# SamShue/EKF_SLAM

Measured on AMD Instinct MI355X. Metric: EKF update-steps/sec at N landmarks; HBM GB/s on (I−KH)P vs roofline, higher is better.
Workload: dtype f64

## Files before the change

ekf_slam_amd/csrc/downdate.h:

```cpp
#pragma once

template <typename TS, int T, int kSlab>
__global__ __launch_bounds__(kBlock) void k_downdate(const TS *__restrict__ tiles, TS *__restrict__ dst,
                                                     const int2 *__restrict__ work, int64_t nwork,
                                                     const double *__restrict__ Kp, const double *__restrict__ Gp,
                                                     int64_t pair_stride, int pstart, int pcap, int npairs, TileMap tm) {
    using V2 = typename Vec2<TS>::type;
    constexpr int kPairsPerRow = T / 2;
    constexpr int kRowsPerPass = kBlock / kPairsPerRow;
    constexpr int kSlabsPerTile = T / kSlab;
    constexpr int kPasses = (kSlab + kRowsPerPass - 1) / kRowsPerPass;
    constexpr bool kExact = kRowsPerPass * kPasses == kSlab;
    static_assert(kPasses <= 8, "slab too tall for the register tile");
    const int tid = threadIdx.x;
    const int cp = tid % kPairsPerRow;
    const int r0 = tid / kPairsPerRow;
    const int64_t nitems = nwork * kSlabsPerTile;
    for (int64_t it0 = blockIdx.x; it0 < nitems; it0 += gridDim.x) {
        const int64_t it = tm.reverse ? nitems - 1 - it0 : it0;
        const int64_t w = it / kSlabsPerTile;
        const int slab = (int)(it - w * kSlabsPerTile);
        const int2 ij = work[w];
        const int64_t toff = tm.tile_offset(ij.x, ij.y) + (int64_t)slab * kSlab * T;
        const TS *__restrict__ tp = tiles + toff;
// ... 28 lines not shown
        for (int p = 0; p < kPasses; ++p) {
            const int r = r0 + p * kRowsPerPass;
            if (kExact || r < kSlab) {
                V2 o;
                o.x = (TS)v[p].x; o.y = (TS)v[p].y;
                *reinterpret_cast<V2 *>(td + r * T + 2 * cp) = o;
            }
        }
    }
}

template <typename TS> struct Lane16;
template <> struct Lane16<double> { using type = double2; static constexpr int kCols = 2; };
template <> struct Lane16<float>  { using type = float4;  static constexpr int kCols = 4; };
__device__ __forceinline__ void lane16_unpack(const double2 &t, double *v) { v[0] = t.x; v[1] = t.y; }
__device__ __forceinline__ void lane16_unpack(const float4 &t, double *v) { v[0] = t.x; v[1] = t.y; v[2] = t.z; v[3] = t.w; }
__device__ __forceinline__ void lane16_pack(const double *v, double2 &t) { t.x = v[0]; t.y = v[1]; }
__device__ __forceinline__ void lane16_pack(const double *v, float4 &t) {
    t.x = (float)v[0]; t.y = (float)v[1]; t.z = (float)v[2]; t.w = (float)v[3];
}
__device__ __forceinline__ double lane16_get(const double2 &t, int q) { return q == 0 ? t.x : t.y; }
__device__ __forceinline__ double lane16_get(const float4 &t, int q) { return (double)(q == 0 ? t.x : q == 1 ? t.y : q == 2 ? t.z : t.w); }

__device__ __attribute__((noinline)) void extract_next_row(double *__restrict__ send, int jm, int Ij, int tI, int tJ, int r, int c0, int ncols,
                                                           int T, int world, int rank, double v0, double v1, double v2, double v3) {
    const uint32_t wd = (uint32_t)world;
    const int k0 = (int)(((uint32_t)rank + wd - (uint32_t)Ij % wd) % wd);
    const bool rowtile = tI == Ij, coltile = tJ == Ij, diag = rowtile && coltile;
    for (int q = 0; q < ncols; ++q) {
        const int cc = c0 + q;
        const double val = q == 0 ? v0 : q == 1 ? v1 : q == 2 ? v2 : v3;
        if (rowtile && (r == jm || r == jm + 1)) {
            const int a = r - jm;
            if (!diag || cc <= jm) {
                const int64_t e = (int64_t)((tJ - k0) / world) * T + cc;
                send[2 * e + a] = val;
            }
            if (diag && a == 1 && (cc == jm || cc == jm + 1)) {
                const int64_t e = (int64_t)((Ij - k0) / world) * T + jm + 1;
                send[2 * e + (cc - jm)] = val;
            }
        }
        if (coltile && (cc == jm || cc == jm + 1) && (tI > Ij || r > jm + 1)) {
            const int64_t e = (int64_t)((tI - k0) / world) * T + r;
            send[2 * e + (cc - jm)] = val;
        }
    }
}

struct NoNextRow {};
template <bool kNext> struct NextRowParam { using type = NoNextRow; };
template <> struct NextRowParam<true> { using type = NextRow; };

template <typename TS, int T, int kSlab, bool kXcd, bool kNext = false>
__global__ __launch_bounds__(kBlock) void k_downdate_w(const TS *__restrict__ tiles, TS *__restrict__ dst,
                                                       const int2 *__restrict__ work, int64_t nwork,
                                                       const double *__restrict__ Kp, const double *__restrict__ Gp,
                                                       int64_t pair_stride, int pstart, int pcap, int npairs, TileMap tm,
                                                       typename NextRowParam<kNext>::type nx) {
    using VL = typename Lane16<TS>::type;
    constexpr int kCols = Lane16<TS>::kCols;
    constexpr int kLanesPerRow = T / kCols;
    constexpr int kRowsPerInstr = 64 / kLanesPerRow;
    constexpr int kRowsPerWave = kSlab / 4;
    constexpr int kPasses = kRowsPerWave / kRowsPerInstr;
    constexpr int kSlabsPerTile = T / kSlab;
    static_assert(kLanesPerRow == 64 || kLanesPerRow == 32, "tile edge / storage type combination not supported");
    static_assert(kPasses >= 1 && kPasses <= 8 && kPasses * kRowsPerInstr * 4 == kSlab, "bad slab");
    const int lane = threadIdx.x & 63;
    const int wave = __builtin_amdgcn_readfirstlane(threadIdx.x >> 6);
    const int sub = lane / kLanesPerRow;
    const int cl = lane % kLanesPerRow;
    const int64_t nitems = (kXcd ? 8 : 1) * nwork * kSlabsPerTile;
    const int64_t nv = nwork * kSlabsPerTile;
    for (int64_t it = blockIdx.x; it < nitems; it += gridDim.x) {
        const int64_t vf = kXcd ? (it >> 3) : it;
        const int64_t vi = tm.reverse ? nv - 1 - vf : vf;
        const int64_t w = vi / kSlabsPerTile;
        const int slab = (int)(vi - w * kSlabsPerTile);
        const int2 ij = work[kXcd ? (it & 7) * nwork + w : w];
        if (kXcd && ij.x < 0) continue;
        const int row0 = slab * kSlab + wave * kRowsPerWave;
        const int64_t toff = tm.tile_offset(ij.x, ij.y) + (int64_t)(row0 + sub) * T + kCols * cl;
        const TS *__restrict__ tp = tiles + toff;
        TS *__restrict__ td = dst + toff;
        double v[kPasses][kCols];
#pragma unroll
        for (int p = 0; p < kPasses; ++p) {
            const VL t = *reinterpret_cast<const VL *>(tp + (int64_t)p * kRowsPerInstr * T);
            lane16_unpack(t, v[p]);
        }
        const int64_t gcol = (int64_t)ij.y * T + kCols * cl;
        const int64_t krow = (int64_t)ij.x * T + row0;
        for (int i = 0; i < npairs; ++i) {
            const int64_t so = (int64_t)ring_slot(pstart, i, pcap) * pair_stride;
            const double2 *__restrict__ g2 = reinterpret_cast<const double2 *>(Gp + so) + gcol;
            const double2 *__restrict__ k2 = reinterpret_cast<const double2 *>(Kp + so) + krow;
            double2 g[kCols];
#pragma unroll
            for (int q = 0; q < kCols; ++q) g[q] = g2[q];
#pragma unroll
            for (int p = 0; p < kPasses; ++p) {
                double2 k = k2[p * kRowsPerInstr];
                if (kRowsPerInstr == 2) { const double2 k1 = k2[p * 2 + 1]; if (sub) k = k1; }
#pragma unroll
                for (int q = 0; q < kCols; ++q) v[p][q] = rank2_apply(v[p][q], k, g[q]);
            }
        }
        VL stored[kPasses];
#pragma unroll
        for (int p = 0; p < kPasses; ++p) {
            lane16_pack(v[p], stored[p]);
            *reinterpret_cast<VL *>(td + (int64_t)p * kRowsPerInstr * T) = stored[p];
        }
        if constexpr (kNext) {
            const int Ij = (int)(nx.j >> tm.shift);
            if (__builtin_expect(ij.x == Ij || ij.y == Ij, 0)) {
#pragma unroll
                for (int p = 0; p < kPasses; ++p) {
                    double vv[4] = { 0.0, 0.0, 0.0, 0.0 };
#pragma unroll
                    for (int q = 0; q < kCols; ++q) vv[q] = lane16_get(stored[p], q);
                    extract_next_row(nx.send, (int)(nx.j & (T - 1)), Ij, ij.x, ij.y, row0 + sub + p * kRowsPerInstr, kCols * cl, kCols, T,
                                     tm.world, tm.rank, vv[0], vv[1], vv[2], vv[3]);
                }
            }
        }
    }
}
```

ekf_slam_amd/csrc/host/handle.h:

```cpp
#pragma once
#include "../../../include/ekfslam.h"
#include <hip/hip_runtime.h>
#include <dlfcn.h>
#include <cstdio>
#include <cstdlib>
#include <algorithm>
#include <cmath>
#include <cstring>
#include <new>
#include <string>
#include <vector>

#include "../device_math.h"
#include "../flush32_pipe.h"
#include "../kernels.h"
#include "../layout.h"

struct KernelTimer {
    bool enabled = false;
    std::vector<hipEvent_t> ev;
    size_t used = 0;
};

struct ekf_handle {
// ... 174 lines not shown
    void *q = nullptr;
    const size_t bytes = (count ? count : 1) * sizeof(Tp);
    hipError_t e = hipMalloc(&q, bytes);
    if (e != hipSuccess) return e;
    e = hipMemset(q, 0, bytes);
    if (e != hipSuccess) return e;
    h->allocs.push_back(q);
    h->bytes += (int64_t)bytes;
    *p = (Tp *)q;
    return hipSuccess;
}

template <typename Tp>
hipError_t halloc(ekf_handle *h, Tp **p, size_t bytes, unsigned flags) {
    const hipError_t e = hipHostMalloc((void **)p, bytes, flags);
    if (e == hipSuccess) h->pinned.push_back(*p);
    return e;
}
hipError_t new_event(ekf_handle *h, hipEvent_t *ev) {
    const hipError_t e = hipEventCreateWithFlags(ev, hipEventDisableTiming);
    if (e == hipSuccess) h->events.push_back(*ev);
    return e;
}

struct DevTemp {
    void **p;
    template <typename Tp> explicit DevTemp(Tp **q) : p((void **)q) {}
    ~DevTemp() { if (*p) hipFree(*p); }
};

template <typename Tp>
int32_t stage_alloc(ekf_handle *h, Tp **area, size_t bytes, hipEvent_t *ev) {
    if (!*area) HIPCHK(h, halloc(h, area, bytes ? bytes : 16, hipHostMallocDefault));
    if (!*ev) HIPCHK(h, new_event(h, ev));
    return EKF_OK;
}
int32_t stage_wait(ekf_handle *h, hipEvent_t ev, bool &busy) { if (busy) { HIPCHK(h, hipEventSynchronize(ev)); busy = false; } return EKF_OK; }
int32_t stage_uploaded(ekf_handle *h, hipEvent_t ev, bool &busy) { HIPCHK(h, hipEventRecord(ev, h->stream)); busy = true; return EKF_OK; }

inline int64_t n_mm(const ekf_handle *h) { return 2 * h->N; }
inline bool decided_mode(const ekf_handle *h) { return h->cfg.mode == EKF_MODE_UC && h->cfg.device_assoc == 4; }
inline int64_t unsettled(const ekf_handle *h) { return decided_mode(h) ? (int64_t)(h->lrec_head - h->lrec_tail) : 0; }
inline int64_t n_hi(const ekf_handle *h) { return h->N + unsettled(h); }
inline size_t elt_size(const ekf_handle *h) { return h->storage == EKF_STORE_F64 ? 8 : 4; }

int32_t use_device(ekf_handle *h) {
    HIPCHK(h, hipSetDevice(h->cfg.device));
    return EKF_OK;
}

struct TimedLaunch {
    hipStream_t s;
    KernelTimer *t;
    hipEvent_t stop = nullptr;
    TimedLaunch(ekf_handle *h, int which) : TimedLaunch(h, which, h->stream) {}
    TimedLaunch(ekf_handle *h, int which, hipStream_t on) : s(on), t(&h->timers[which]) {
        if (!t->enabled) { t = nullptr; return; }
        if (t->used + 2 > t->ev.size()) {
            hipEvent_t a, b;
            if (hipEventCreate(&a) != hipSuccess || hipEventCreate(&b) != hipSuccess) { t = nullptr; return; }
            t->ev.push_back(a); t->ev.push_back(b);
        }
        hipEventRecord(t->ev[t->used], s);
        stop = t->ev[t->used + 1];
        t->used += 2;
    }
    ~TimedLaunch() { if (t) hipEventRecord(stop, s); }
};

#define TIMED(h, which, call) do { TimedLaunch tl_((h), (which)); HIPCHK((h), call); } while (0)

void colmajor2(const double R[4], double &r00, double &r01, double &r10, double &r11) {
    r00 = R[0]; r10 = R[1]; r01 = R[2]; r11 = R[3];
}
}
```

ekf_slam_amd/csrc/host/passes.h:

```cpp
#pragma once
namespace {
int32_t refresh_work(ekf_handle *h) {
    const int64_t nt = ekf_tiles_for(2 * n_hi(h), h->T);
    if (nt == h->ws[h->ws_cur].rows) return EKF_OK;
    const int32_t to = h->ws_pass == h->ws_cur ? h->ws_cur ^ 1 : h->ws_cur;
    ekf_handle::WorkSet &ws = h->ws[to];
    const size_t b_work = (size_t)h->work_cap * sizeof(int2), b_xcd = 8 * b_work, b_segs = (size_t)h->segs_cap * sizeof(int4);
    if (!h->wl_stage) h->wl_stage_bytes = b_work + b_xcd + b_segs;
    int32_t rc = stage_alloc(h, &h->wl_stage, h->wl_stage_bytes, &h->ev_wl);
    if (!rc) rc = stage_wait(h, h->ev_wl, h->wl_busy);
    if (rc) return rc;
    int2 *w = reinterpret_cast<int2 *>(h->wl_stage);
    int2 *flat = reinterpret_cast<int2 *>(h->wl_stage + b_work);
    int4 *segs = reinterpret_cast<int4 *>(h->wl_stage + b_work + b_xcd);
    size_t nw = 0;
    REQUIRE(h, h->st.tm.slots_for_rows(nt) <= h->work_cap, EKF_ERR_STATE, "work list overflow");
    for (int64_t I = 0; I < nt; ++I)
        for (int64_t J = 0; J <= I; ++J)
            if (h->st.tm.mine(I, J)) w[nw++] = make_int2((int)I, (int)J);
    if (nw) HIPCHK(h, hipMemcpyAsync(ws.work, w, nw * sizeof(int2), hipMemcpyHostToDevice, h->stream));
    ws.nwork = (int64_t)nw;
    ws.rows = nt;

    static const int S = std::max(1, ekf_tune_int("EKF_SUPERTILE", 8));
// ... 6 lines not shown
            for (int64_t I = si * S; I < nt && I < (si + 1) * S; ++I)
                for (int64_t J = sj * S; J <= I && J < (sj + 1) * S; ++J)
                    if (h->st.tm.mine(I, J)) sp.tiles.push_back(make_int2((int)I, (int)J));
            if (!sp.tiles.empty()) supers.push_back(std::move(sp));
        }
    static const int order = ekf_tune_int("EKF_XCD_ORDER", 1);
    std::vector<int2> stream[8];
    if (order == 0) {
        std::stable_sort(supers.begin(), supers.end(), [](const Super &a, const Super &b) { return a.tiles.size() > b.tiles.size(); });
        for (const Super &sp : supers) {
            int best = 0;
            for (int x = 1; x < 8; ++x) if (stream[x].size() < stream[best].size()) best = x;
            stream[best].insert(stream[best].end(), sp.tiles.begin(), sp.tiles.end());
        }
    } else {
        std::vector<int2> flat_order;
        flat_order.reserve(nw);
        for (const Super &sp : supers) flat_order.insert(flat_order.end(), sp.tiles.begin(), sp.tiles.end());
        const size_t tot = flat_order.size();
        for (int x = 0; x < 8; ++x)
            stream[x].assign(flat_order.begin() + (tot * x) / 8, flat_order.begin() + (tot * (x + 1)) / 8);
    }
    size_t len = 0;
    for (int x = 0; x < 8; ++x) len = std::max(len, stream[x].size());
    REQUIRE(h, (int64_t)(8 * len) <= 8 * h->work_cap, EKF_ERR_STATE, "XCD work list overflow");
    std::fill(flat, flat + 8 * len, make_int2(-1, -1));
    for (int x = 0; x < 8; ++x) std::copy(stream[x].begin(), stream[x].end(), flat + x * len);
    if (len) HIPCHK(h, hipMemcpyAsync(ws.xcd, flat, 8 * len * sizeof(int2), hipMemcpyHostToDevice, h->stream));
    ws.xcd_len = (int64_t)len;
    if (ws.segs) {
        std::vector<int4> sg;
        const int64_t nsegs = ekf_pipe32::build_strip_segments(h->st.tm, nt, sg);
        REQUIRE(h, (int64_t)sg.size() <= h->segs_cap, EKF_ERR_STATE, "strip work list overflow");
        if (!sg.empty()) {
            std::copy(sg.begin(), sg.end(), segs);
            HIPCHK(h, hipMemcpyAsync(ws.segs, segs, sg.size() * sizeof(int4), hipMemcpyHostToDevice, h->stream));
        }
        ws.nsegs = nsegs;
        ws.cols = nt * h->T;
    }
    TRY(stage_uploaded(h, h->ev_wl, h->wl_busy));
    h->ws_cur = to;
    h->ws_unordered = true;
    return EKF_OK;
}

const PassAux *pass_aux(const ekf_handle *h, const ekf_handle::WorkSet &ws, PassAux &out) {
    if (!ws.segs) return nullptr;
    out = h->aux;
    out.segs = ws.segs; out.nsegs = ws.nsegs; out.cols = ws.cols;
    return &out;
}

PassJob pass_job(const ekf_handle *h, const ekf_handle::WorkSet &ws, void *dst, PassAux &ax) {
    PassJob job = {};
    job.dst = dst;
    job.work = ws.work; job.nwork = ws.nwork; job.work_xcd = ws.xcd; job.xcd_len = ws.xcd_len;
    job.pstart = h->pstart; job.npairs = h->npend;
    job.grid_cap = h->grid_cap; job.arith = h->cfg.pass_arith;
    job.aux = pass_aux(h, ws, ax);
    return job;
}

int32_t create_worklists(ekf_handle *h) {
    for (auto &ws : h->ws) {
        if (h->cfg.pass_arith != EKF_ARITH_F64) HIPCHK(h, dalloc(h, &ws.segs, (size_t)h->segs_cap));
        HIPCHK(h, dalloc(h, &ws.work, (size_t)h->work_cap));
        HIPCHK(h, dalloc(h, &ws.xcd, (size_t)h->work_cap * 8));
    }
    return EKF_OK;
}

int32_t retire_inflight(ekf_handle *h) {
    if (!h->inflight) return EKF_OK;
    if (h->appended_inflight) {
        if (!h->ev_rows) HIPCHK(h, new_event(h, &h->ev_rows));
        HIPCHK(h, hipEventRecord(h->ev_rows, h->stream));
        HIPCHK(h, hipStreamWaitEvent(h->flush_stream, h->ev_rows, 0));
        if (decided_mode(h)) {
            const int64_t *hi = unsettled(h) > 0 ? h->d_nring + h->nrow % ekf_handle::kNRing : nullptr;
            HIPCHK(h, launch_copy_rows_dev(h->st.tm, h->tilebuf[h->base], h->tilebuf[h->base ^ 1], 2 * h->inflight_N, 2 * n_hi(h), h->inflight_dn,
                                           hi, h->storage, h->flush_stream));
        } else
            HIPCHK(h, launch_copy_rows(h->st.tm, h->tilebuf[h->base], h->tilebuf[h->base ^ 1], 2 * h->inflight_N, 2 * h->N, h->storage, h->flush_stream));
        HIPCHK(h, hipEventRecord(h->ev_flushed, h->flush_stream));
        h->appended_inflight = false;
    }
    HIPCHK(h, hipStreamWaitEvent(h->stream, h->ev_flushed, 0));
    h->ws_pass = -1;
    h->base ^= 1;
    h->st.tiles = h->tilebuf[h->base];
    h->pstart = (h->pstart + h->nfrozen) % h->st.pcap;
    h->npend -= h->nfrozen;
    h->nfrozen = 0;
    h->inflight = false;
    tiles_changed(h);
    return EKF_OK;
}

void next_pass_direction(ekf_handle *h) {
    const int force = h->cfg.pass_direction == 1 ? 0 : h->cfg.pass_direction == 2 ? 1 : -1;
    constexpr int64_t kCacheBytes = 256ll << 20;
    const int64_t nt = ekf_tiles_for(2 * n_hi(h), h->T);
    const int64_t store = nt * (nt + 1) / 2 / std::max(1, h->cfg.world) * (int64_t)h->T * h->T * (h->storage == EKF_STORE_F64 ? 8 : 4);
    const bool alternate = force >= 0 ? force != 0 : store > kCacheBytes;
    h->st.tm.reverse = alternate ? (h->st.tm.reverse ^ 1) : 0;
}

int32_t flush_pending(ekf_handle *h, bool batch_done = false) {
    TRY(retire_inflight(h));
    if (h->npend == 0) return EKF_OK;
    TRY(refresh_work(h));
    next_pass_direction(h);
    bool extracted = false;
    const int64_t hint = h->hint_idx;
    bool pn = false, pn_side = false;
    if (batch_done && !h->pn_idx.empty()) {
        if (h->sharded && !h->pending && h->pn_N == h->N && (h->comm || h->xhook)) {
            const int32_t m = (int32_t)h->pn_idx.size();
            const int64_t slab = slab_for(h, n_mm(h));
            TIMED(h, EKF_KERNEL_ROWPANEL, launch_rowpanel_next(h->st, h->pn_idx.data(), m, n_mm(h), h->pstart, h->npend, h->send, slab, h->storage,
                  h->stream));
            tiles_changed(h);
            h->pf_idx = h->pn_idx; h->pf_m = m; h->pf_slab = slab; h->pf_N = h->N;
            h->x_count = (int64_t)m * slab;
            static const int pn_side_stream = ekf_tune_int("EKF_PN_SIDE_STREAM", 0);
            if (h->comm) {
                pn_side = pn_side_stream != 0;
                if (pn_side && !h->xchg_stream) {
                    HIPCHK(h, hipStreamCreateWithFlags(&h->xchg_stream, hipStreamNonBlocking));
                    HIPCHK(h, new_event(h, &h->ev_pn_ready));
                    HIPCHK(h, new_event(h, &h->ev_pn_done));
                }
                if (pn_side) {
                    HIPCHK(h, hipEventRecord(h->ev_pn_ready, h->stream));
                    HIPCHK(h, hipStreamWaitEvent(h->xchg_stream, h->ev_pn_ready, 0));
                }
                const hipStream_t xs = pn_side ? h->xchg_stream : h->stream;
                const int r = g_rccl.AllGather(h->send, h->recv, (size_t)h->x_count,  8, h->comm, xs);
                if (r != 0) return fail(h, EKF_ERR_COMM, g_rccl.GetErrorString(r));
                HIPCHK(h, store_panels(h, xs));
                if (pn_side) HIPCHK(h, hipEventRecord(h->ev_pn_done, h->xchg_stream));
            } else {
                TRY(exchange_bracket(h, 2));
                HIPCHK(h, store_panels(h, h->stream));
            }
            pn = true;
        }
        drop_announced(h);
    }
    {
        NextRow nx = { -1, nullptr };
        if (h->sharded && h->npend == 1 && !h->pending && hint >= 0 && hint < h->N) {
            nx.j = 2 * hint;
            nx.send = corr_send(h, slab_for(h, n_mm(h)));
        }
        TimedLaunch tl(h, EKF_KERNEL_DOWNDATE);
        const ekf_handle::WorkSet &ws = h->ws[h->ws_cur];
        PassAux ax;
        PassJob job = pass_job(h, ws, h->st.tiles, ax);
        job.nx = nx.j >= 0 ? &nx : nullptr;
        HIPCHK(h, launch_downdate(h->st, job, h->storage, h->stream, h->dd_kernel, &extracted));
        h->dd_pairs = h->npend;
    }
    h->npend = 0;
    h->pstart = 0;
    h->pf_valid = pn;
    if (pn_side) HIPCHK(h, hipStreamWaitEvent(h->stream, h->ev_pn_done, 0));
    h->nx_valid = extracted && !pn;
    if (extracted) { h->nx_idx = hint; h->nx_N = h->N; }
    return EKF_OK;
}

int32_t batch_complete(ekf_handle *h) {
    if (!h->async_flush) return flush_pending(h,  true);
    HIPCHK(h, hipEventRecord(h->ev_pairs, h->stream));
    h->ws_unordered = false;
    TRY(retire_inflight(h));
    TRY(refresh_work(h));
    HIPCHK(h, hipStreamWaitEvent(h->flush_stream, h->ev_pairs, 0));
    if (h->ws_unordered) HIPCHK(h, hipStreamWaitEvent(h->flush_stream, h->ev_wl, 0));
    {
        TimedLaunch tl(h, EKF_KERNEL_DOWNDATE, h->flush_stream);
        next_pass_direction(h);
        const ekf_handle::WorkSet &ws = h->ws[h->ws_cur];
        PassAux ax;
        HIPCHK(h, launch_downdate(h->st, pass_job(h, ws, h->tilebuf[h->base ^ 1], ax), h->storage, h->flush_stream, h->dd_kernel));
        h->dd_pairs = h->npend;
    }
    HIPCHK(h, hipEventRecord(h->ev_flushed, h->flush_stream));
    h->nfrozen = h->npend;
    h->inflight = true;
    h->ws_pass = h->ws_cur;
    h->inflight_N = h->N;
    h->inflight_dn = unsettled(h) > 0 ? h->d_nring + h->nrow % ekf_handle::kNRing : nullptr;
    h->appended_inflight = false;
    return EKF_OK;
}

int32_t create_passes(ekf_handle *h, const hipDeviceProp_t &prop) {
    const ekf_config &cfg = h->cfg;
    const int32_t T = h->T;
    const int64_t ldm = h->st.ldm, slots = h->work_cap, nt_cap = ldm / T;
    char *tiles = nullptr;
    HIPCHK(h, dalloc(h, &tiles, (size_t)slots * T * T * elt_size(h)));
    h->st.tiles = tiles;
    h->tilebuf[0] = tiles;
    h->async_flush = cfg.async_flush != 0;
    if (h->async_flush) {
        char *tiles2 = nullptr;
        HIPCHK(h, dalloc(h, &tiles2, (size_t)slots * T * T * elt_size(h)));
        h->tilebuf[1] = tiles2;
        int reserve = ekf_tune_int("EKF_ASYNC_RESERVE_CUS", cfg.pass_arith == EKF_ARITH_SPLIT3 ? 64 : 32);
        const int ncu = prop.multiProcessorCount;
        if (reserve > 0 && ncu == 256) {
            if (reserve > 128) reserve = 128;
            uint32_t mask[8];
            for (int w = 0; w < 8; ++w) mask[w] = 0xffffffffu;
            int taken = 0;
            for (int b = 0; b < 16 && taken < reserve; ++b)
                for (int a = 0; a < 8 && taken < reserve; ++a) {
                    const int bit = 32 * a + 8 * (b & 3) + ((a + (b >> 2)) & 7);
                    if (mask[bit >> 5] & (1u << (bit & 31))) { mask[bit >> 5] &= ~(1u << (bit & 31)); ++taken; }
                }
            HIPCHK(h, hipExtStreamCreateWithCUMask(&h->flush_stream, 8, mask));
            h->flush_cus = ncu - taken;
        } else {
            int lo = 0, hi = 0;
            HIPCHK(h, hipDeviceGetStreamPriorityRange(&lo, &hi));
            HIPCHK(h, hipStreamCreateWithPriority(&h->flush_stream, hipStreamNonBlocking, lo));
        }
        HIPCHK(h, new_event(h, &h->ev_pairs));
        HIPCHK(h, new_event(h, &h->ev_flushed));
    }
    h->batch = cfg.batch < 1 ? 1 : cfg.batch;
    h->cfg.batch = h->batch;
    h->st.pair_stride = 2 * ldm;
    h->st.pcap = h->async_flush ? 2 * h->batch : h->batch;
    HIPCHK(h, dalloc(h, &h->st.Gp, (size_t)(2 * ldm) * h->st.pcap * 2));
    h->st.Kp = h->st.Gp + (size_t)(2 * ldm) * h->st.pcap;
// ... 23 lines not shown
```

ekf_slam_amd/csrc/kernel_args.h:

```cpp
#pragma once
#include <stdint.h>

#include "layout.h"

struct DevState {
    double *x[2];
    double *prr[2];
    double *strip[2];
    void   *tiles;
    double *s;
    double *Gp;
    double *Kp;
    float  *Gp32;
    float  *Kp32;
    int64_t pair_stride;
    int32_t pcap;
    double *small;
    int64_t ldm;
    TileMap tm;
    double *diag[2];
    int32_t dcur;
};

struct PredictArgs {
    double u0, u1, C;
    int64_t n_mm;
    int32_t cur;
};

struct AssocHostPartial;

struct DevLoopArgs {
    const AssocHostPartial *parts_in;
    AssocHostPartial *rec;
    AssocHostPartial *parts_out;
    int32_t nblk_in, seq_in;
    int32_t seq_rec, seq_out;
    double z0, z1, z2;
    double R00, R01, R10, R11;
    double s_cost, s_thresh, w_pos;
    const int64_t *dn_in;
    int64_t *dn_out;
    int64_t n_known;
    const double *loc;
    int64_t loc_base;
    double u0, u1;
    int32_t *abort;
    int32_t scan_id;
};

struct AppendArgs {
    double u0, u1;
    double R00, R01, R10, R11;
    double pos0, pos1, signature;
    int64_t N;
    int32_t cur;
};

constexpr int kAppendModelMax = 32;
struct AppendModelEntry {
    double z0, z1;
    double R00, R01, R10, R11;
    double signature;
    int32_t model, pad;
};
struct AppendModelArgs {
    int64_t N;
    int32_t m;
    int32_t cur;
    AppendModelEntry e[kAppendModelMax];
};

struct JoinMapArgs {
    int64_t N;
    int64_t M;
    double signature_offset;
// ... 233 lines not shown
```

ekf_slam_amd/csrc/kernels.h:

```cpp
#pragma once
#include <hip/hip_runtime.h>
#include <stdint.h>

#include "device_math.h"
#include "assign_math.h"
#include "kernel_args.h"
#include "layout.h"

#ifdef EKF_TUNING
#include <stdlib.h>
inline int ekf_tune_int(const char *name, int dflt) { const char *v = getenv(name); return v ? atoi(v) : dflt; }
#else
constexpr int ekf_tune_int(const char *, int dflt) { return dflt; }
#endif

hipError_t launch_predict(const DevState &st, const PredictArgs &a, int storage, hipStream_t s);

hipError_t launch_predict_model(const DevState &st, const PredictModelArgs &a, hipStream_t s);

hipError_t launch_append(const DevState &st, const AppendArgs &a, int storage, hipStream_t s, const DevLoopArgs *dl = nullptr,
                         const PredictArgs *fused_predict = nullptr);

hipError_t launch_append_model(const DevState &st, const AppendModelArgs &a, int storage, hipStream_t s);

// ... 38 lines not shown
struct alignas(16) AssocHostPartial {
    double  min_ll;
    int32_t index;
    int32_t tag;
};
#if defined(__HIPCC__)
__host__ __device__
#endif
inline uint32_t assoc_part_mix(uint32_t ll_lo, uint32_t ll_hi, uint32_t index) {
    uint32_t m = ll_lo * 0x9E3779B1u ^ (ll_hi + 0x7F4A7C15u) * 0x85EBCA6Bu ^ (index + 0x165667B1u) * 0xC2B2AE35u;
    m ^= m >> 15; m *= 0x2C1B3C6Du; m ^= m >> 13;
    return m;
}

constexpr int kAssocBlock = 256;

hipError_t launch_associate(const DevState &st, const AssocArgs &a, double *pos_cost, double *sig_cost,
                            AssocDecision *partial, int *ticket, AssocDecision *decision, AssocHostPartial *host_partials, int seq,
                            double *cand, int storage, hipStream_t s, const PredictArgs *fused_predict = nullptr);
hipError_t launch_associate_devn(const DevState &st, const AssocArgs &a, AssocHostPartial *host_partials, int seq, int storage,
                                 hipStream_t s, const PredictArgs *fused_predict);
hipError_t launch_assoc_merge(const DevState &st, const double *recv, int world, int64_t count, int64_t N, bool want_costs,
                              double *pos_cost, AssocDecision *decision, AssocDecision *host_decision, int seq, hipStream_t s);

hipError_t launch_assoc_model(const DevState &st, const AssocModelArgs &a, ekfm::Match2 *partials, ekfm::Match2 *out, double *d2_all,
                              hipStream_t s);

hipError_t launch_assign_model(const DevState &st, const AssocModelArgs &a, ekfm::Match2 *partials, ekfm::CandList *lists, ekfm::CandList *sel,
                               AssignResult *res, hipStream_t s);
hipError_t launch_assign_lists(const DevState &st, const AssocModelArgs &a, ekfm::Match2 *partials, ekfm::CandList *lists, ekfm::CandList *sel,
                               AssignResult *res, hipStream_t s);

struct NextRow { int64_t j; double *send; };
struct PassAux {
    const int4 *segs;
    int64_t nsegs;
    float *dump;
    int grid;
    int64_t cols;
    uint16_t *Kb3, *Gb3;
};
size_t pass_split_plane_elems(int64_t ldm);
struct PassJob {
    void *dst;
    const int2 *work;
    int64_t nwork;
    const int2 *work_xcd;
    int64_t xcd_len;
    int pstart, npairs;
    int grid_cap;
    int arith;
    const PassAux *aux;
    const NextRow *nx;
};
hipError_t launch_downdate(const DevState &st, const PassJob &job, int storage, hipStream_t s, char *kname, bool *extracted = nullptr);
hipError_t launch_copy_rows(const TileMap &tm, const void *src, void *dst, int64_t r0, int64_t r1, int storage, hipStream_t s);
hipError_t launch_copy_rows_dev(const TileMap &tm, const void *src, void *dst, int64_t r0, int64_t r1, const int64_t *n_lo,
                                const int64_t *n_hi, int storage, hipStream_t s);

hipError_t launch_compact_tiles(const TileMap &tm, const void *src, void *dst, const int2 *work, int64_t ntiles, const int32_t *src_of,
                                int storage, hipStream_t s);
hipError_t launch_compact_state(const DevState &st, int cur, const int32_t *src_of, int64_t N_old, double *s_out, hipStream_t s);
hipError_t launch_constrain_probe(const DevState &st, int cur, int64_t ai, int64_t aj, double *out, int storage, hipStream_t s);
hipError_t launch_gather_constrain(const DevState &st, const ConstrainArgs &a, int storage, hipStream_t s);
hipError_t launch_gather_constrain_chain(const DevState &st, const ConstrainArgs &a, double *rec, int storage, hipStream_t s);
hipError_t launch_merge_pass(const DevState &st, void *dst, const int2 *work, int64_t ntiles, const int32_t *src_of, int npairs,
                             int storage, hipStream_t s, char *kname);
hipError_t launch_nearest(const DevState &st, int cur, int64_t N, const double R[4], NearestEntry *out, int storage, hipStream_t s);

hipError_t launch_gather_linear(const DevState &st, const LinearArgs &a, double *rec, int64_t *cnt, int storage, hipStream_t s);
hipError_t launch_linear_probe(const DevState &st, const LinearArgs &a, double *rec, int storage, hipStream_t s);

hipError_t launch_gather_model(const DevState &st, const ModelArgs &a, double *rec, int64_t *cnt, int storage, hipStream_t s);
hipError_t launch_model_probe(const DevState &st, const ModelArgs &a, double *rec, int storage, hipStream_t s);
hipError_t launch_gather_model_assigned(const DevState &st, const AssignedModelArgs &a, const AssignedRecord *slot, double *rec, int64_t *cnt,
                                        int storage, hipStream_t s);
hipError_t launch_gather_model_iter(const DevState &st, const IterModelArgs &a, double *rec, int64_t *cnt, double *itrec, int storage, hipStream_t s);
hipError_t launch_model_iter_probe(const DevState &st, const IterModelArgs &a, double *rec, double *itrec, int storage, hipStream_t s);

hipError_t launch_joint_innovation(const DevState &st, const JointArgs &a, const int64_t *hyp, int nh, JointRecord *out, double *d2_prefix,
                                   double *nu, double *S, int storage, hipStream_t s);

hipError_t launch_joint_search_prepare(const DevState &st, const JointArgs &a, const ekfm::CandList *sel, const int64_t *match,
                                       JointSearchStore *store, JointSearchOut *out, hipStream_t s);
hipError_t launch_joint_search_level(const DevState &st, const JointSearchArgs &a, const JointSearchLevelArgs &la, const ekfm::CandList *sel,
                                     JointSearchStore *store, JointSearchOut *out, int which, int storage, hipStream_t s);

hipError_t launch_joint_factor(const DevState &st, const JointArgs &a, const int64_t *hyp, JointBlock *blk, JointRecord *out, double *nu, double *S,
                               int storage, hipStream_t s);
hipError_t launch_joint_factor_iter(const DevState &st, const JointArgs &a, const JointIterArgs &ia, const int64_t *hyp, JointBlock *blk,
                                    JointRecord *out, double *itrec, double *nu, double *S, int storage, hipStream_t s);
hipError_t launch_gather_joint(const DevState &st, const JointUpdateArgs &a, const JointBlock *blk, int storage, hipStream_t s);

hipError_t launch_unpack_dense(const DevState &st, int cur, int64_t n_mm, double *dense, int storage, hipStream_t s);
hipError_t launch_pack_dense(const DevState &st, int cur, int64_t n_mm, const double *dense, int storage, hipStream_t s);
hipError_t launch_get_block(const DevState &st, int cur, int64_t r0, int64_t c0, int64_t nr, int64_t nc,
                            double *out, int storage, hipStream_t s);
hipError_t launch_get_diag_blocks(const DevState &st, int cur, int64_t N, double *out, int storage, hipStream_t s);
hipError_t launch_lowrank(const DevState &st, int cur, int64_t n_mm, const int2 *work, int64_t nwork, const double *d,
                          const double *U, int64_t k, int storage, hipStream_t s);
constexpr int kDigestGrid = 2048;
constexpr int kDigestDoubles = 4 + 3 * kDigestGrid;
hipError_t launch_digest(const DevState &st, int cur, int64_t n_mm, const int2 *work, int64_t nwork, double *out,
                         int storage, hipStream_t s);
```

ekf_slam_amd/csrc/launch/passes.h:

```cpp
#pragma once

size_t pass_split_plane_elems(int64_t ldm) { return ekf_pipe32::split_plane_elems(ldm); }

namespace {
hipError_t allow_dynamic_lds(const void *fn, size_t bytes, std::atomic<uint64_t> &done) {
    int dev = 0;
    hipError_t e = hipGetDevice(&dev);
    if (e != hipSuccess) return e;
    const uint64_t bit = 1ull << (dev & 63);
    if (done.load(std::memory_order_acquire) & bit) return hipSuccess;
    e = hipFuncSetAttribute(fn, hipFuncAttributeMaxDynamicSharedMemorySize, (int)bytes);
    if (e == hipSuccess) done.fetch_or(bit, std::memory_order_release);
    return e;
}

template <typename TS_, int kT, int kSlab> struct PassShape { using TS = TS_; static constexpr int T = kT, slab = kSlab; };
template <typename... S> struct PassShapes {};
using ValuShapes = PassShapes<
    PassShape<double, 16, 16>, PassShape<double, 32, 16>, PassShape<double, 32, 32>,
    PassShape<double, 64, 8>, PassShape<double, 64, 16>, PassShape<double, 64, 32>, PassShape<double, 64, 64>,
    PassShape<double, 128, 4>, PassShape<double, 128, 8>, PassShape<double, 128, 16>, PassShape<double, 128, 32>,
    PassShape<float, 16, 16>, PassShape<float, 32, 32>, PassShape<float, 64, 64>, PassShape<float, 128, 8>, PassShape<float, 128, 64>,
    PassShape<float, 256, 4>, PassShape<float, 256, 8>, PassShape<float, 256, 16>, PassShape<float, 256, 32>>;

template <typename F, typename... S> bool with_shape(PassShapes<S...>, const ekf_pass::PassInstance &p, F &&f) {
    return (((int)sizeof(typename S::TS) == p.elt && S::T == p.T && S::slab == p.slab ? (f(S{}), true) : false) || ...);
}
}

hipError_t launch_downdate(const DevState &st, const PassJob &job, int storage, hipStream_t s, char *kname, bool *extracted) {
    using namespace ekf_pass;
    if (extracted) *extracted = false;
    if (job.nwork <= 0 || job.npairs <= 0) return hipSuccess;
    static const int slab1 = ekf_tune_int("EKF_DOWNDATE_SLAB", 0);
    static const int slabm = ekf_tune_int("EKF_DOWNDATE_SLAB_BATCH", 0);
    static const PassKnobs knobs = { ekf_tune_int("EKF_FLUSH_MFMA", 1) != 0, ekf_tune_int("EKF_FLUSH_MFMA_SWITCH", 30), ekf_tune_int("EKF_FLUSH_HALF_MAX", 12),
                                     ekf_tune_int("EKF_PASS_STRIP", 1) != 0, ekf_tune_int("EKF_FLUSH_XCD", 1) != 0 };
    const PassAux *aux = job.aux;
    const int T = st.tm.T, pstart = job.pstart, npairs = job.npairs;
    PassQuery q = { storage == 0 ? 8 : 4, T, npairs, job.arith,  job.work_xcd && job.xcd_len > 0,
                     aux && aux->segs && aux->nsegs > 0,  aux && aux->Kb3 && aux->Gb3,  job.nx && job.nx->j >= 0,
                     npairs > 1 ? slabm : slab1 };
    PassInstance p = select_pass(q, knobs);
    static std::atomic<uint64_t> split_ok{0}, strip_ok{0};
    if (p.family == kSplit3 && allow_dynamic_lds((const void *)ekf_pipe32::k_flush_split3<2>, ekf_pipe32::lds_bytes_split(), split_ok) != hipSuccess) {
        q.planes = false;
        p = select_pass(q, knobs);
    }
    if (p.family == kStrip32 && allow_dynamic_lds((const void *)ekf_pipe32::k_flush_strip32<8>, ekf_pipe32::lds_bytes_strip<8>(), strip_ok) != hipSuccess) {
        q.strip_list = false;
        p = select_pass(q, knobs);
    }

    auto flush = [&](auto kernel, auto ts, auto *Kp, auto *Gp, int rows, int cols) {
        using TS = decltype(ts);
        hipLaunchKernelGGL(kernel, dim3(clamp_grid(8 * job.xcd_len * (T / rows) * (T / cols), job.grid_cap)), dim3(kBlock), 0, s,
                           (const TS *)st.tiles, (TS *)job.dst, job.work_xcd, job.xcd_len, Kp, Gp, st.pair_stride, pstart, st.pcap, npairs, st.tm);
    };
    switch (p.family) {
        case kInvalid: return hipErrorInvalidValue;
        case kSplit3:
            hipLaunchKernelGGL(ekf_pipe32::k_split_pairs, dim3((unsigned)(aux->cols / 256), ekf_pipe32::kKB, 2), dim3(256), 0, s, (const float *)st.Kp32,
                               (const float *)st.Gp32, aux->Kb3, aux->Gb3, st.pair_stride, st.ldm, aux->cols, pstart, st.pcap, npairs);
            hipLaunchKernelGGL((ekf_pipe32::k_flush_split3<2>), dim3((unsigned)aux->grid), dim3(512), ekf_pipe32::lds_bytes_split(), s,
                               (const float *)st.tiles, (float *)job.dst, aux->segs, aux->nsegs, (const uint16_t *)aux->Kb3, (const uint16_t *)aux->Gb3, st.ldm,
                               st.tm, aux->dump);
            break;
        case kStrip32:
            hipLaunchKernelGGL((ekf_pipe32::k_flush_strip32<8>), dim3((unsigned)aux->grid), dim3(512), ekf_pipe32::lds_bytes_strip<8>(), s,
                               (const float *)st.tiles, (float *)job.dst, aux->segs, aux->nsegs, (const float *)st.Kp32, (const float *)st.Gp32, st.pair_stride,
                               st.ldm, pstart, st.pcap, npairs, st.tm, aux->dump, (unsigned long long *)nullptr);
            break;
        case kMfma32:
            if (p.early) flush(k_flush_mfma32<256, 4, 2, 3, true>, float{}, st.Kp32, st.Gp32, 128, 128);
            else flush(k_flush_mfma32<256, 4, 2, 3>, float{}, st.Kp32, st.Gp32, 128, 128);
            break;
        case kMfma64:
            if (p.elt == 4) {
                if (p.chunk == 4) flush(k_flush_mfma<float, 256, 4>, float{}, st.Kp, st.Gp, 64, 128);
                else flush(k_flush_mfma<float, 256, 8>, float{}, st.Kp, st.Gp, 64, 128);
            } else if (p.cols == 64) flush(k_flush_mfma<double, 128, 4, 64, 5>, double{}, st.Kp, st.Gp, 64, 64);
            else if (p.chunk == 4) flush(k_flush_mfma<double, 128, 4>, double{}, st.Kp, st.Gp, 64, 128);
            else flush(k_flush_mfma<double, 128, 8>, double{}, st.Kp, st.Gp, 64, 128);
            break;
        case kDowndateW:
        case kDowndate: {
            const bool built = with_shape(ValuShapes{}, p, [&](auto shape) {
                using TS = typename decltype(shape)::TS;
                constexpr int kT = decltype(shape)::T, kSlab = decltype(shape)::slab, kLanes = kT / Lane16<TS>::kCols;
                const TS *src = (const TS *)st.tiles;
                TS *dst = (TS *)job.dst;
                const dim3 grid(clamp_grid(job.nwork * (kT / kSlab), job.grid_cap)), grid_xcd(clamp_grid(8 * job.xcd_len * (kT / kSlab), job.grid_cap));
                if constexpr (kLanes != 64 && kLanes != 32) {
                    hipLaunchKernelGGL((k_downdate<TS, kT, kSlab>), grid, dim3(kBlock), 0, s, src, dst, job.work, job.nwork, st.Kp, st.Gp,
                                       st.pair_stride, pstart, st.pcap, npairs, st.tm);
                } else {
                    auto per_row = [&](auto kernel, dim3 g, const int2 *list, int64_t n, auto next) {
                        hipLaunchKernelGGL(kernel, g, dim3(kBlock), 0, s, src, dst, list, n, st.Kp, st.Gp, st.pair_stride, pstart, st.pcap, npairs, st.tm, next);
                    };
                    if (p.xcd) per_row(k_downdate_w<TS, kT, kSlab, true>, grid_xcd, job.work_xcd, job.xcd_len, NoNextRow{});
                    else if (p.rowpanel) per_row(k_downdate_w<TS, kT, kSlab, false, true>, grid, job.work, job.nwork, *job.nx);
                    else per_row(k_downdate_w<TS, kT, kSlab, false>, grid, job.work, job.nwork, NoNextRow{});
                }
            });
            if (!built) return hipErrorInvalidValue;
            if (extracted) *extracted = p.rowpanel;
            break;
        }
    }
    if (kname) snprintf(kname, 64, "%s", p.name);
    return hipGetLastError();
}

namespace {
template <typename Launch>
hipError_t copy_tile_rows(const TileMap &tm, int64_t r0, int64_t r1, int storage, Launch &&launch) {
    if (r1 <= r0) return hipSuccess;
    const int T = tm.T;
    if (T > kBlock * (storage == 0 ? 2 : 4)) return hipErrorInvalidValue;
    hipError_t e = hipSuccess;
    for (int64_t I = r0 >> tm.shift; I <= (r1 - 1) >> tm.shift; ++I) {
        const int64_t lo = std::max<int64_t>(r0, I * T) - I * T, hi = std::min<int64_t>(r1, (I + 1) * T) - I * T;
        const int64_t slot0 = tm.row_base(I), nslots = tm.row_base(I + 1) - slot0;
        if (nslots <= 0 || hi <= lo) continue;
        const int lanes = T / (storage == 0 ? 2 : 4), per_wg = kBlock / lanes > 0 ? kBlock / lanes : 1;
        const hipError_t ei = launch(dim3((unsigned)cdiv(nslots * (hi - lo), per_wg)), slot0, nslots, (int)lo, (int)(hi - lo), I);
        if (ei != hipSuccess) e = ei;
    }
    return e;
}
}

hipError_t launch_copy_rows(const TileMap &tm, const void *src, void *dst, int64_t r0, int64_t r1, int storage, hipStream_t s) {
    return copy_tile_rows(tm, r0, r1, storage, [&](dim3 grid, int64_t slot0, int64_t nslots, int lo, int n, int64_t) {
        return with_storage(storage, [&](auto ts) {
            using TS = decltype(ts);
            hipLaunchKernelGGL(k_copy_tile_rows<TS>, grid, dim3(kBlock), 0, s, (const TS *)src, (TS *)dst, slot0, nslots, lo, n, tm.T);
        });
    });
}

hipError_t launch_copy_rows_dev(const TileMap &tm, const void *src, void *dst, int64_t r0, int64_t r1, const int64_t *n_lo,
                                const int64_t *n_hi, int storage, hipStream_t s) {
    return copy_tile_rows(tm, r0, r1, storage, [&](dim3 grid, int64_t slot0, int64_t nslots, int lo, int n, int64_t I) {
        return with_storage(storage, [&](auto ts) {
            using TS = decltype(ts);
            hipLaunchKernelGGL(k_copy_tile_rows_dev<TS>, grid, dim3(kBlock), 0, s, (const TS *)src, (TS *)dst, slot0, nslots, lo, n, tm.T,
                               I * tm.T, r0, r1, n_lo, n_hi);
        });
    });
}
```

Before: 1940.

## Trim padded rows in the last tile row and widen downdate workgroups

The wide downdate kernel now takes a PassGeom that enumerates work items so the last tile row only covers the rows that actually exist, skipping padded rows of the (I−KH)P update. Guarded loads and stores use a magic-number division to map those items. Workgroups default to 8 wavefronts covering more rows per item. Kernel timing can now use hipExtLaunchKernelGGL events tied to the launch itself. The cost is extra index arithmetic and branches per item, plus a new launch path.

Result: no change. 1940 (-0.0%).

```diff
diff --git a/ekf_slam_amd/csrc/downdate.h b/ekf_slam_amd/csrc/downdate.h
--- a/ekf_slam_amd/csrc/downdate.h
+++ b/ekf_slam_amd/csrc/downdate.h
@@ -104,42 +104,60 @@
 template <bool kNext> struct NextRowParam { using type = NoNextRow; };
 template <> struct NextRowParam<true> { using type = NextRow; };
 
-template <typename TS, int T, int kSlab, bool kXcd, bool kNext = false>
-__global__ __launch_bounds__(kBlock) void k_downdate_w(const TS *__restrict__ tiles, TS *__restrict__ dst,
-                                                       const int2 *__restrict__ work, int64_t nwork,
-                                                       const double *__restrict__ Kp, const double *__restrict__ Gp,
-                                                       int64_t pair_stride, int pstart, int pcap, int npairs, TileMap tm,
-                                                       typename NextRowParam<kNext>::type nx) {
+template <typename TS, int T, int kSlab, bool kXcd, bool kNext = false, int kWaves = 4>
+__global__ __launch_bounds__(64 * kWaves) void k_downdate_w(PassGeom pg, const TS *__restrict__ tiles, TS *__restrict__ dst,
+                                                            const int2 *__restrict__ work, int64_t nwork,
+                                                            const double *__restrict__ Kp, const double *__restrict__ Gp,
+                                                            int64_t pair_stride, int pstart, int pcap, int npairs, TileMap tm,
+                                                            typename NextRowParam<kNext>::type nx) {
     using VL = typename Lane16<TS>::type;
     constexpr int kCols = Lane16<TS>::kCols;
     constexpr int kLanesPerRow = T / kCols;
     constexpr int kRowsPerInstr = 64 / kLanesPerRow;
     constexpr int kRowsPerWave = kSlab / 4;
     constexpr int kPasses = kRowsPerWave / kRowsPerInstr;
-    constexpr int kSlabsPerTile = T / kSlab;
+    constexpr int kItemRows = kRowsPerWave * kWaves;
+    constexpr int kSlabsPerTile = T / kItemRows;
+    constexpr bool kGuard = !kXcd && (kPasses > 1 || kNext);
     static_assert(kLanesPerRow == 64 || kLanesPerRow == 32, "tile edge / storage type combination not supported");
     static_assert(kPasses >= 1 && kPasses <= 8 && kPasses * kRowsPerInstr * 4 == kSlab, "bad slab");
+    static_assert((kWaves == 4 || kWaves == 8 || kWaves == 16) && kItemRows <= T && T % kItemRows == 0, "bad workgroup width");
+    static_assert(!kXcd || kWaves == 4, "the per-XCD streams are walked by 4-wavefront workgroups");
     const int lane = threadIdx.x & 63;
     const int wave = __builtin_amdgcn_readfirstlane(threadIdx.x >> 6);
     const int sub = lane / kLanesPerRow;
     const int cl = lane % kLanesPerRow;
-    const int64_t nitems = (kXcd ? 8 : 1) * nwork * kSlabsPerTile;
-    const int64_t nv = nwork * kSlabsPerTile;
+    const int64_t nv = kXcd ? nwork * kSlabsPerTile : (int64_t)pg.nitems;
+    const int64_t nitems = (kXcd ? 8 : 1) * nv;
     for (int64_t it = blockIdx.x; it < nitems; it += gridDim.x) {
-        const int64_t vf = kXcd ? (it >> 3) : it;
-        const int64_t vi = tm.reverse ? nv - 1 - vf : vf;
-        const int64_t w = vi / kSlabsPerTile;
-        const int slab = (int)(vi - w * kSlabsPerTile);
+        int64_t w;
+        int slab, rows = T;
+        if constexpr (kXcd) {
+            const int64_t vf = it >> 3, vi = tm.reverse ? nv - 1 - vf : vf;
+            w = vi / kSlabsPerTile;
+            slab = (int)(vi - w * kSlabsPerTile);
+        } else {
+            const uint32_t vi = tm.reverse ? pg.nitems - 1 - (uint32_t)it : (uint32_t)it;
+            const int over = (int)vi - (int)pg.full_items;
+            const bool last = over >= 0;
+            const uint32_t u = (uint32_t)over, q = __umulhi(2 * u + 1, pg.last_magic);
+            w = last ? pg.nfull + q : vi / kSlabsPerTile;
+            slab = (int)(last ? u - q * pg.last_items : vi % kSlabsPerTile);
+            rows = last ? (int)pg.last_rows : T;
+        }
         const int2 ij = work[kXcd ? (it & 7) * nwork + w : w];
         if (kXcd && ij.x < 0) continue;
-        const int row0 = slab * kSlab + wave * kRowsPerWave;
+        const int row0 = slab * kItemRows + wave * kRowsPerWave;
+        const int left = rows - (row0 + sub);
+        if (!kXcd && !kNext && left <= 0) continue;
         const int64_t toff = tm.tile_offset(ij.x, ij.y) + (int64_t)(row0 + sub) * T + kCols * cl;
         const TS *__restrict__ tp = tiles + toff;
         TS *__restrict__ td = dst + toff;
         double v[kPasses][kCols];
 #pragma unroll
         for (int p = 0; p < kPasses; ++p) {
-            const VL t = *reinterpret_cast<const VL *>(tp + (int64_t)p * kRowsPerInstr * T);
+            VL t = {};
+            if (!kGuard || p * kRowsPerInstr < left) t = *reinterpret_cast<const VL *>(tp + (int64_t)p * kRowsPerInstr * T);
             lane16_unpack(t, v[p]);
         }
         const int64_t gcol = (int64_t)ij.y * T + kCols * cl;
@@ -163,7 +181,8 @@
 #pragma unroll
         for (int p = 0; p < kPasses; ++p) {
             lane16_pack(v[p], stored[p]);
-            *reinterpret_cast<VL *>(td + (int64_t)p * kRowsPerInstr * T) = stored[p];
+            if (!kGuard || p * kRowsPerInstr < left) *reinterpret_cast<VL *>(td + (int64_t)p * kRowsPerInstr * T) = stored[p];
+            else stored[p] = VL{};
         }
         if constexpr (kNext) {
             const int Ij = (int)(nx.j >> tm.shift);
diff --git a/ekf_slam_amd/csrc/host/handle.h b/ekf_slam_amd/csrc/host/handle.h
--- a/ekf_slam_amd/csrc/host/handle.h
+++ b/ekf_slam_amd/csrc/host/handle.h
@@ -250,20 +250,22 @@
 struct TimedLaunch {
     hipStream_t s;
     KernelTimer *t;
-    hipEvent_t stop = nullptr;
+    bool bracket;
+    hipEvent_t start = nullptr, stop = nullptr;
     TimedLaunch(ekf_handle *h, int which) : TimedLaunch(h, which, h->stream) {}
-    TimedLaunch(ekf_handle *h, int which, hipStream_t on) : s(on), t(&h->timers[which]) {
+    TimedLaunch(ekf_handle *h, int which, hipStream_t on, bool bracket_ = true) : s(on), t(&h->timers[which]), bracket(bracket_) {
         if (!t->enabled) { t = nullptr; return; }
         if (t->used + 2 > t->ev.size()) {
             hipEvent_t a, b;
             if (hipEventCreate(&a) != hipSuccess || hipEventCreate(&b) != hipSuccess) { t = nullptr; return; }
             t->ev.push_back(a); t->ev.push_back(b);
         }
-        hipEventRecord(t->ev[t->used], s);
+        start = t->ev[t->used];
         stop = t->ev[t->used + 1];
         t->used += 2;
+        if (bracket) hipEventRecord(start, s);
     }
-    ~TimedLaunch() { if (t) hipEventRecord(stop, s); }
+    ~TimedLaunch() { if (t && bracket) hipEventRecord(stop, s); }
 };
 
 #define TIMED(h, which, call) do { TimedLaunch tl_((h), (which)); HIPCHK((h), call); } while (0)
diff --git a/ekf_slam_amd/csrc/host/passes.h b/ekf_slam_amd/csrc/host/passes.h
--- a/ekf_slam_amd/csrc/host/passes.h
+++ b/ekf_slam_amd/csrc/host/passes.h
@@ -82,9 +82,12 @@
     return &out;
 }
 
-PassJob pass_job(const ekf_handle *h, const ekf_handle::WorkSet &ws, void *dst, PassAux &ax) {
+PassJob pass_job(const ekf_handle *h, const ekf_handle::WorkSet &ws, void *dst, PassAux &ax, const TimedLaunch &tl) {
     PassJob job = {};
     job.dst = dst;
+    job.ev_start = tl.t ? tl.start : nullptr; job.ev_stop = tl.t ? tl.stop : nullptr;
+    const int64_t rows = 2 * n_hi(h);
+    job.rows = ekf_tiles_for(rows, h->T) == ws.rows ? rows : 0;
     job.work = ws.work; job.nwork = ws.nwork; job.work_xcd = ws.xcd; job.xcd_len = ws.xcd_len;
     job.pstart = h->pstart; job.npairs = h->npend;
     job.grid_cap = h->grid_cap; job.arith = h->cfg.pass_arith;
@@ -185,10 +188,10 @@
             nx.j = 2 * hint;
             nx.send = corr_send(h, slab_for(h, n_mm(h)));
         }
-        TimedLaunch tl(h, EKF_KERNEL_DOWNDATE);
+        TimedLaunch tl(h, EKF_KERNEL_DOWNDATE, h->stream,  false);
         const ekf_handle::WorkSet &ws = h->ws[h->ws_cur];
         PassAux ax;
-        PassJob job = pass_job(h, ws, h->st.tiles, ax);
+        PassJob job = pass_job(h, ws, h->st.tiles, ax, tl);
         job.nx = nx.j >= 0 ? &nx : nullptr;
         HIPCHK(h, launch_downdate(h->st, job, h->storage, h->stream, h->dd_kernel, &extracted));
         h->dd_pairs = h->npend;
@@ -211,11 +214,11 @@
     HIPCHK(h, hipStreamWaitEvent(h->flush_stream, h->ev_pairs, 0));
     if (h->ws_unordered) HIPCHK(h, hipStreamWaitEvent(h->flush_stream, h->ev_wl, 0));
     {
-        TimedLaunch tl(h, EKF_KERNEL_DOWNDATE, h->flush_stream);
+        TimedLaunch tl(h, EKF_KERNEL_DOWNDATE, h->flush_stream,  false);
         next_pass_direction(h);
         const ekf_handle::WorkSet &ws = h->ws[h->ws_cur];
         PassAux ax;
-        HIPCHK(h, launch_downdate(h->st, pass_job(h, ws, h->tilebuf[h->base ^ 1], ax), h->storage, h->flush_stream, h->dd_kernel));
+        HIPCHK(h, launch_downdate(h->st, pass_job(h, ws, h->tilebuf[h->base ^ 1], ax, tl), h->storage, h->flush_stream, h->dd_kernel));
         h->dd_pairs = h->npend;
     }
     HIPCHK(h, hipEventRecord(h->ev_flushed, h->flush_stream));
diff --git a/ekf_slam_amd/csrc/kernel_args.h b/ekf_slam_amd/csrc/kernel_args.h
--- a/ekf_slam_amd/csrc/kernel_args.h
+++ b/ekf_slam_amd/csrc/kernel_args.h
@@ -22,6 +22,15 @@
     int32_t dcur;
 };
 
+struct PassGeom {
+    uint32_t nitems;
+    uint32_t full_items;
+    uint32_t nfull;
+    uint32_t last_items;
+    uint32_t last_rows;
+    uint32_t last_magic;
+};
+
 struct PredictArgs {
     double u0, u1, C;
     int64_t n_mm;
diff --git a/ekf_slam_amd/csrc/kernels.h b/ekf_slam_amd/csrc/kernels.h
--- a/ekf_slam_amd/csrc/kernels.h
+++ b/ekf_slam_amd/csrc/kernels.h
@@ -114,6 +114,8 @@
     int arith;
     const PassAux *aux;
     const NextRow *nx;
+    int64_t rows;
+    hipEvent_t ev_start, ev_stop;
 };
 hipError_t launch_downdate(const DevState &st, const PassJob &job, int storage, hipStream_t s, char *kname, bool *extracted = nullptr);
 hipError_t launch_copy_rows(const TileMap &tm, const void *src, void *dst, int64_t r0, int64_t r1, int storage, hipStream_t s);
diff --git a/ekf_slam_amd/csrc/launch/passes.h b/ekf_slam_amd/csrc/launch/passes.h
--- a/ekf_slam_amd/csrc/launch/passes.h
+++ b/ekf_slam_amd/csrc/launch/passes.h
@@ -1,4 +1,5 @@
 #pragma once
+#include <hip/hip_ext.h>
 
 size_t pass_split_plane_elems(int64_t ldm) { return ekf_pipe32::split_plane_elems(ldm); }
 
@@ -26,12 +27,34 @@
 template <typename F, typename... S> bool with_shape(PassShapes<S...>, const ekf_pass::PassInstance &p, F &&f) {
     return (((int)sizeof(typename S::TS) == p.elt && S::T == p.T && S::slab == p.slab ? (f(S{}), true) : false) || ...);
 }
+
+constexpr int kPassWaves = 8;
+template <typename F> void with_pass_width(F &&f) {
+#ifdef EKF_TUNING
+    static const int waves = ekf_tune_int("EKF_PASS_WAVES", kPassWaves);
+    if (waves == 4) return f(std::integral_constant<int, 4>{});
+#endif
+    f(std::integral_constant<int, kPassWaves>{});
+}
+
+struct PassBracket {
+    hipStream_t s;
+    hipEvent_t start, stop;
+    bool armed = false;
+    void begin() { armed = true; hipEventRecord(start, s); }
+    ~PassBracket() { if (armed) hipEventRecord(stop, s); }
+};
 }
 
 hipError_t launch_downdate(const DevState &st, const PassJob &job, int storage, hipStream_t s, char *kname, bool *extracted) {
     using namespace ekf_pass;
     if (extracted) *extracted = false;
-    if (job.nwork <= 0 || job.npairs <= 0) return hipSuccess;
+    const bool timed = job.ev_start && job.ev_stop;
+    PassBracket bracket = { s, job.ev_start, job.ev_stop };
+    if (job.nwork <= 0 || job.npairs <= 0) {
+        if (timed) bracket.begin();
+        return hipSuccess;
+    }
     static const int slab1 = ekf_tune_int("EKF_DOWNDATE_SLAB", 0);
     static const int slabm = ekf_tune_int("EKF_DOWNDATE_SLAB_BATCH", 0);
     static const PassKnobs knobs = { ekf_tune_int("EKF_FLUSH_MFMA", 1) != 0, ekf_tune_int("EKF_FLUSH_MFMA_SWITCH", 30), ekf_tune_int("EKF_FLUSH_HALF_MAX", 12),
@@ -51,6 +74,25 @@
         q.strip_list = false;
         p = select_pass(q, knobs);
     }
+    static const bool tie_events = ekf_tune_int("EKF_PASS_TIMING_TIED", 1) != 0;
+    const bool tied = timed && tie_events && p.family == kDowndateW;
+    if (timed && !tied) bracket.begin();
+    static const bool tight = ekf_tune_int("EKF_PASS_TIGHT", 1) != 0;
+    int64_t nlast = 0;
+    int last_rows = T;
+    if (tight && job.rows > 0) {
+        const int64_t nt = st.tm.tiles_for(job.rows);
+        int64_t mine = nt;
+        if (st.tm.world > 1) {
+            mine = 0;
+            for (int64_t J = 0; J < nt; ++J) mine += st.tm.mine(nt - 1, J);
+        }
+        const bool whole_list = st.tm.world > 1 ? mine <= job.nwork : st.tm.slots_for_rows(nt) == job.nwork;
+        if (whole_list && job.rows < nt * T && mine * T * T < (1ll << 29)) {
+            nlast = mine;
+            last_rows = (int)(job.rows - (nt - 1) * T);
+        }
+    }
 
     auto flush = [&](auto kernel, auto ts, auto *Kp, auto *Gp, int rows, int cols) {
         using TS = decltype(ts);
@@ -85,25 +127,51 @@
             break;
         case kDowndateW:
         case kDowndate: {
+            bool fits = true;
             const bool built = with_shape(ValuShapes{}, p, [&](auto shape) {
                 using TS = typename decltype(shape)::TS;
                 constexpr int kT = decltype(shape)::T, kSlab = decltype(shape)::slab, kLanes = kT / Lane16<TS>::kCols;
                 const TS *src = (const TS *)st.tiles;
                 TS *dst = (TS *)job.dst;
-                const dim3 grid(clamp_grid(job.nwork * (kT / kSlab), job.grid_cap)), grid_xcd(clamp_grid(8 * job.xcd_len * (kT / kSlab), job.grid_cap));
                 if constexpr (kLanes != 64 && kLanes != 32) {
+                    const dim3 grid(clamp_grid(job.nwork * (kT / kSlab), job.grid_cap));
                     hipLaunchKernelGGL((k_downdate<TS, kT, kSlab>), grid, dim3(kBlock), 0, s, src, dst, job.work, job.nwork, st.Kp, st.Gp,
                                        st.pair_stride, pstart, st.pcap, npairs, st.tm);
                 } else {
-                    auto per_row = [&](auto kernel, dim3 g, const int2 *list, int64_t n, auto next) {
-                        hipLaunchKernelGGL(kernel, g, dim3(kBlock), 0, s, src, dst, list, n, st.Kp, st.Gp, st.pair_stride, pstart, st.pcap, npairs, st.tm, next);
+                    auto geom = [&](int item_rows, bool whole) {
+                        PassGeom g = {};
+                        const int64_t nfull = job.nwork - nlast, full_items = nfull * (kT / item_rows);
+                        g.last_items = (uint32_t)(whole ? kT / item_rows : (last_rows + item_rows - 1) / item_rows);
+                        g.last_magic = (uint32_t)(((1ull << 31) + g.last_items - 1) / g.last_items);
+                        g.last_rows = (uint32_t)last_rows;
+                        const int64_t nitems = full_items + nlast * g.last_items;
+                        fits = fits && nitems < (1ll << 31);
+                        g.nfull = (uint32_t)nfull; g.full_items = (uint32_t)full_items; g.nitems = (uint32_t)nitems;
+                        return g;
                     };
-                    if (p.xcd) per_row(k_downdate_w<TS, kT, kSlab, true>, grid_xcd, job.work_xcd, job.xcd_len, NoNextRow{});
-                    else if (p.rowpanel) per_row(k_downdate_w<TS, kT, kSlab, false, true>, grid, job.work, job.nwork, *job.nx);
-                    else per_row(k_downdate_w<TS, kT, kSlab, false>, grid, job.work, job.nwork, NoNextRow{});
+                    auto per_row = [&](auto kernel, int waves, int64_t items, const int2 *list, int64_t n, const PassGeom &g, auto next) {
+                        if (!fits) return;
+                        const dim3 grid(clamp_grid(items, job.grid_cap)), block(64 * waves);
+                        if (tied) hipExtLaunchKernelGGL(kernel, grid, block, 0, s, job.ev_start, job.ev_stop, 0, g, src, dst, list, n, st.Kp, st.Gp,
+                                                        st.pair_stride, pstart, st.pcap, npairs, st.tm, next);
+                        else hipLaunchKernelGGL(kernel, grid, block, 0, s, g, src, dst, list, n, st.Kp, st.Gp, st.pair_stride, pstart, st.pcap, npairs,
+                                                st.tm, next);
+                    };
+                    if (p.xcd) per_row(k_downdate_w<TS, kT, kSlab, true>, 4, 8 * job.xcd_len * (kT / kSlab), job.work_xcd, job.xcd_len, PassGeom{}, NoNextRow{});
+                    else with_pass_width([&](auto width) {
+                        constexpr int kW = kSlab / 4 * decltype(width)::value <= kT ? decltype(width)::value : 4;
+                        constexpr int kItemRows = kSlab / 4 * kW;
+                        if (p.rowpanel) {
+                            const PassGeom g = geom(kItemRows, true);
+                            per_row(k_downdate_w<TS, kT, kSlab, false, true, kW>, kW, g.nitems, job.work, job.nwork, g, *job.nx);
+                        } else {
+                            const PassGeom g = geom(kItemRows, false);
+                            per_row(k_downdate_w<TS, kT, kSlab, false, false, kW>, kW, g.nitems, job.work, job.nwork, g, NoNextRow{});
+                        }
+                    });
                 }
             });
-            if (!built) return hipErrorInvalidValue;
+            if (!built || !fits) return hipErrorInvalidValue;
             if (extracted) *extracted = p.rowpanel;
             break;
         }
```
